# xxayt/MGSV

Hardware: AMD Instinct MI355X
Metric: video-music pairs/s fwd+bwd at B=64 (full training step); sub-objects: retrieval sim-matrix GB/s, eval forward pairs/s (higher is better)
Workload: dtype bf16; 1 GPU; BASELINE.json configs[2]: B=64/GPU, T_v=30, T_a=512, D=512, train mode (dropout on), f32 master weights + Adam, f32 gradient accumulation; global_batch=64, launch=tape

## Files before the change

include/made_hip.h:

```cpp
#ifndef MADE_HIP_H
#define MADE_HIP_H

#include <stdint.h>

#ifdef __cplusplus
extern "C" {
#endif

#define MADE_ABI_VERSION 8

enum MadeDtype { MADE_F32 = 0, MADE_BF16 = 1 };

enum MadeAct {
    MADE_ACT_NONE = 0,
    MADE_ACT_RELU = 1,
    MADE_ACT_GELU = 2,
    MADE_ACT_QUICKGELU = 3,
    MADE_ACT_SIGMOID = 4
};

enum MadeGate {
    MADE_GATE_NONE = 0,
    MADE_GATE_RELU_OUT = 1,
    MADE_GATE_GELU_Z = 2,
// ... 475 lines not shown
                        int64_t B, int64_t T, int64_t F, void* stream);
int made_posbn_relu_bwd(const void* x, int32_t x_dtype, int64_t ldx, const void* y, int32_t y_dtype, int64_t ldy,
                        const void* dy, int32_t dy_dtype, int64_t lddy, const float* weight, const float* save_mean,
                        const float* save_rstd, int32_t batch_stats, void* dx, int32_t dx_dtype, int64_t lddx,
                        float* dweight, float* dbias, int64_t B, int64_t T, int64_t F, void* stream);

int made_set_criterion_bwd(const float* pred_logits, const float* pred_spans, const float* targets,
                           const int64_t* pred_idx, const int64_t* tgt_idx, const int32_t* count,
                           const float* proj_queries, const float* vid_sum, const float* empty_weight,
                           int64_t n_layers, int64_t B, int64_t Q, int64_t G, int64_t Dc, int32_t fg_label,
                           float temperature, const float* weights, const float* upstream,
                           float* d_logits, float* d_spans, int64_t ld_out, int32_t through_sigmoid,
                           float* d_proj_queries, float* d_vid_sum, void* stream);

#define MADE_ADAM_MAX_GROUPS 4
#define MADE_ADAM_NORM_BLOCKS 1024
typedef struct MadeAdamGroup { int64_t begin, end; float lr; float max_norm; } MadeAdamGroup;
int made_adam_step(float* param, const float* grad, float* exp_avg, float* exp_avg_sq, int64_t n,
                   const MadeAdamGroup* groups, int32_t n_groups, float beta1, float beta2, float eps, int64_t step,
                   float grad_scale, float* norm_ws, void* stream);

typedef struct MadeAdamDeviceState { int64_t step; float lr[MADE_ADAM_MAX_GROUPS]; float bc1, bc2_sqrt; } MadeAdamDeviceState;
int made_adam_step_device(float* param, const float* grad, float* exp_avg, float* exp_avg_sq, int64_t n,
                          const MadeAdamGroup* groups, int32_t n_groups, float beta1, float beta2, float eps,
                          MadeAdamDeviceState* state_device, int32_t advance_state, float grad_scale, float* norm_ws, void* stream);

typedef struct MadeRepackDesc {
    const float* src; void* w; void* wt;
    int64_t rows, cols, wt_ld, tile_begin;
    int32_t dtype; int32_t _pad;
} MadeRepackDesc;
int made_repack(const MadeRepackDesc* descs_device, int32_t n_desc, int64_t total_tiles, void* stream);


int made_recall_ranks(const float* sims, int64_t ld, const int32_t* group_id, const int32_t* gt_group, int64_t Nv, int64_t Nm,
                      int64_t n_groups, int32_t* rank_out, int32_t* top1_out, void* stream);

int made_span_iou(const float* pred_logits, const float* pred_spans, const float* gt_moment, const float* m_duration,
                  int64_t N, int64_t Q, int32_t fg_label, float max_m_duration, float* iou_out, float* pred_out, void* stream);

int made_concat_cols(const float* a, int64_t cols_a, const float* c, int64_t cols_c, float* out, int64_t rows, void* stream);


int made_pooled_cosine(const float* anchor, int64_t lda, const void* pooled, int32_t pooled_dtype, float* out, int64_t sa, int64_t sp,
                       int64_t A, int64_t P, int64_t D, void* stream);
int made_scale_exp(const float* x, const float* logit_scale, float* out, int64_t n, void* stream);
int made_span_convert(const float* in, float* out, int64_t N, int32_t mode, void* stream);
int made_span_pairwise(const float* spans1, const float* spans2, float* iou, float* uni, float* giou, float* inter_over_2,
                       int64_t N, int64_t M, void* stream);
int made_span_iou_se(const float* pred_se, const float* gt_moment, const float* m_duration, int64_t N, float max_m_duration,
                     int32_t clamp_to_max, int32_t discounted, float* iou_out, void* stream);


int64_t made_topk_groups_ws_bytes(int64_t Nv, int64_t Nm, int64_t K);
int made_topk_groups(const float* sims, int64_t ld, const int32_t* group_id, int64_t Nv, int64_t Nm, int64_t n_groups,
                     int64_t K, int32_t* idx_out, float* score_out, void* ws, int64_t ws_bytes, void* stream);

int made_gather_pairs(const int32_t* vi, const int32_t* mi, int64_t P, int64_t Nv, int64_t Nm,
                      const void* v_tok, int64_t v_tok_stride, const float* v_mask, int64_t v_mask_stride,
                      const float* v_vec, int64_t v_vec_stride,
                      const void* m_tok, int64_t m_tok_stride, const float* m_mask, int64_t m_mask_stride,
                      const float* m_vec, int64_t m_vec_stride, int64_t Tv, int64_t Ta, int64_t D, int32_t dtype,
                      void* frame_out, int64_t frame_out_stride, void* seg_out, int64_t seg_out_stride,
                      float* fmask_out, float* smask_out, float* video_out, float* music_out, void* stream);


// ... 48 lines not shown
```

mgsv_amd/_lib.py:

```python
from __future__ import annotations

import ctypes as C
import os

_HERE = os.path.dirname(os.path.abspath(__file__))


def variant_env(name: str, default: str = "") -> str:
    if os.environ.get("MADE_DEBUG_VARIANTS", "0") in ("", "0"):
        return default
    return os.environ.get(name, default)


LIB_PATH = os.environ.get("MADE_LIB_PATH") or os.path.join(_HERE, "libmade_hip.so")
ABI_VERSION = 8

F32, BF16 = 0, 1
ACT_NONE, ACT_RELU, ACT_GELU, ACT_QUICKGELU, ACT_SIGMOID = 0, 1, 2, 3, 4
GATE_NONE, GATE_RELU_OUT, GATE_GELU_Z, GATE_QUICKGELU_Z, GATE_SIGMOID_OUT = 0, 1, 2, 3, 4

vp, i64, i32, f32 = C.c_void_p, C.c_int64, C.c_int32, C.c_float

WIDE_PLAN_HEAD, WIDE_PLAN_SAMPLE, WIDE_PLAN_SLOT, WIDE_PLAN_SLOT_BITS = 4, 4, 16, 8

# ... 130 lines not shown

class MadeGemmTNArgs(C.Structure):
    _fields_ = [("A", vp), ("B", vp), ("C", vp), ("ab_dtype", i32), ("c_dtype", i32),
                ("M", i64), ("N", i64), ("K", i64), ("lda", i64), ("ldb", i64), ("ldc", i64),
                ("batch1", i64), ("batch2", i64),
                ("a_zs1", i64), ("a_zs2", i64), ("b_zs1", i64), ("b_zs2", i64), ("c_zs1", i64), ("c_zs2", i64),
                ("row_mask", vp), ("mask_zs1", i64), ("mask_zs2", i64),
                ("alpha", f32), ("accumulate", i32), ("split_m", i64),
                ("colsum", vp), ("colsum_zs1", i64), ("colsum_zs2", i64), ("row_group_valid", vp),
                ("row_index", vp), ("n_rows", vp)]


class MadeGemmTNProblem(C.Structure):
    _fields_ = [("A", vp), ("B", vp), ("C", vp), ("colsum", vp), ("N", i64), ("K", i64), ("lda", i64), ("ldb", i64), ("ldc", i64)]


class MadeGemmTNGroup(C.Structure):
    _fields_ = [("n_problems", i32), ("alpha", f32), ("M", i64), ("split_m", i64), ("row_index", vp), ("n_rows", vp),
                ("p", MadeGemmTNProblem * 8), ("tile_end", i32 * 8), ("tile_size", i32), ("_pad", i32),
                ("workspace", vp), ("workspace_bytes", i64)]


class MadeAdamGroup(C.Structure):
    _fields_ = [("begin", i64), ("end", i64), ("lr", f32), ("max_norm", f32)]


class MadeAdamDeviceState(C.Structure):
    _fields_ = [("step", i64), ("lr", f32 * 4), ("bc1", f32), ("bc2_sqrt", f32)]


class MadeRepackDesc(C.Structure):
    _fields_ = [("src", vp), ("w", vp), ("wt", vp), ("rows", i64), ("cols", i64), ("wt_ld", i64), ("tile_begin", i64),
                ("dtype", i32), ("_pad", i32)]


class MadeFrameDesc(C.Structure):
    _fields_ = [("offset", i64), ("coef", i64), ("H", i32), ("W", i32), ("kh", i32), ("kv", i32)]


class MadeResampleDesc(C.Structure):
    _fields_ = [("offset", i64), ("n", i64), ("taps", i64), ("o", i32), ("m", i32), ("width", i32), ("_pad", i32)]


class MadeAudioSegDesc(C.Structure):
    _fields_ = [("first", i64), ("count", i64)]


SIGNATURES = {
    "made_abi_version": (C.c_int, []),
    "made_set_f32_products": (C.c_int, [C.c_int]),
    "made_get_f32_products": (C.c_int, []),
    "made_last_error": (C.c_char_p, []),
    "made_device_info": (C.c_int, [C.c_char_p, C.c_int, C.POINTER(C.c_int), C.POINTER(C.c_int)]),
    "made_tape_begin": (C.c_int, []),
    "made_tape_end": (C.c_int, [C.POINTER(C.c_uint64)]),
    "made_tape_replay": (C.c_int, [C.c_uint64]),
    "made_tape_free": (C.c_int, [C.c_uint64]),
    "made_tape_interleave": (C.c_int, [C.c_uint64, i32]),
    "made_tape_count": (C.c_int, [C.c_uint64, C.POINTER(i64), C.POINTER(i64), C.POINTER(i64)]),
    "made_tape_replay_range": (C.c_int, [C.c_uint64, i64, i64]),
    "made_tape_op": (C.c_int, [C.c_uint64, i64, C.POINTER(i32), C.POINTER(C.c_uint64), C.POINTER(C.c_uint64), C.POINTER(C.c_uint32)]),
    "made_stream_wait": (C.c_int, [vp, vp]),
    "made_tape_event": (C.c_int, [i32, i32, vp]),
    "made_tape_callback": (C.c_int, [C.CFUNCTYPE(C.c_int, vp), vp]),
    "made_memset_async": (C.c_int, [vp, i32, i64, vp]),
    "made_copy_async": (C.c_int, [vp, vp, i64, vp]),
# ... 12 lines not shown
    "made_layernorm_add": (C.c_int, [vp, i32, i64, vp, vp, vp, i32, i64, vp, i32, i64, vp, i64, i64, i64, f32, vp, vp]),
    "made_cast_mask_rows": (C.c_int, [vp, i64, vp, vp, i32, i64, i64, i64, vp]),
    "made_pack_music_records": (C.c_int, [vp, i32, i64, vp, i64, vp, i64, vp, i32, i64, i64, i64, i64, i64, vp]),
    "made_masked_mean": (C.c_int, [vp, i32, i64, i64, vp, vp, i64, i64, i64, vp]),
    "made_l2norm_rows": (C.c_int, [vp, i32, i64, vp, vp, i32, i64, i64, i64, f32, vp]),
    "made_sine_pe": (C.c_int, [vp, vp, vp, i32, i64, i64, i64, vp]),
    "made_masked_softmax": (C.c_int, [vp, i64, vp, i64, vp, i32, i64, i64, i64, i64, i64, f32, vp]),
    "made_xpool_tail": (C.c_int, [vp, i32, i64, vp, vp, vp, i64, vp, vp, i64, i64, i64, i64, f32, vp]),
    "made_clip_loss": (C.c_int, [vp, i64, i64, vp, f32, i32, vp, vp, vp]),
    "made_hungarian_match": (C.c_int, [vp, vp, vp, i64, i64, i64, i64, i32, f32, f32, f32, vp, i32, vp, vp, vp, vp, vp]),
    "made_attention_bwd": (C.c_int, [C.POINTER(MadeAttnBwdArgs), vp]),
    "made_layernorm_bwd": (C.c_int, [vp, i32, i64, i64, i64, vp, vp, i32, i64, vp, i32, i64, vp, i32, i64, vp, i64,
                                     C.POINTER(MadeDropout), i64, vp, vp, i64, i64, f32, vp, vp]),
    "made_layernorm_bwd2": (C.c_int, [vp, vp, i64, vp, vp, i64, vp, i64, vp, i64, vp, i64, vp, i64, C.POINTER(MadeDropout), i64, i32,
                                      vp, vp, vp, vp, i64, i64, f32, vp]),
    "made_pool_bwd": (C.c_int, [vp, vp, vp, vp, i32, i64, i64, vp, i32, i64, i64, vp, i32, i64, i64, i64, i64, i64, f32, vp]),
    "made_l2norm_bwd": (C.c_int, [vp, i32, i64, vp, i64, i64, vp, i64, i32, vp, i32, i64, i64, i64, f32, vp]),
    "made_clip_loss_bwd": (C.c_int, [vp, i64, i64, vp, f32, vp, vp, vp, vp, i32, vp, vp, vp]),
    "made_xpool_tail_bwd": (C.c_int, [vp, i32, i64, vp, vp, vp, i64, vp, i64, vp, i32, i64, vp, C.POINTER(MadeDropout),
                                      vp, vp, vp, i64, vp, i64, f32, i64, i64, i64, f32, vp]),
    "made_softmax_bwd": (C.c_int, [vp, i64, vp, i64, vp, i64, vp, f32, C.POINTER(MadeDropout), vp, vp, vp, i32, i64, i64,
                                   i64, i64, i64, i64, i64, vp]),
    "made_head_bias": (C.c_int, [vp, i32, i64, vp, vp, i64, i64, i64, vp]),
    "made_head_bias_bwd": (C.c_int, [vp, i32, i64, vp, vp, vp, vp, i64, i64, i64, vp]),
    "made_add3": (C.c_int, [vp, i32, vp, i32, vp, i32, vp, i32, i64, i64, vp]),
    "made_colsum": (C.c_int, [vp, i32, i64, i64, i64, vp, vp]),
    "made_posbn_relu_fwd": (C.c_int, [vp, i32, i64, vp, vp, vp, vp, C.c_float, C.c_float, i32, vp, vp, vp, i32, i64, i64, i64, i64, vp]),
    "made_posbn_relu_bwd": (C.c_int, [vp, i32, i64, vp, i32, i64, vp, i32, i64, vp, vp, vp, i32, vp, i32, i64, vp, vp, i64, i64, i64, vp]),
    "made_set_criterion_bwd": (C.c_int, [vp, vp, vp, vp, vp, vp, vp, vp, vp, i64, i64, i64, i64, i64, i32, f32, vp, vp,
                                         vp, vp, i64, i32, vp, vp, vp]),
    "made_adam_step": (C.c_int, [vp, vp, vp, vp, i64, C.POINTER(MadeAdamGroup), i32, f32, f32, f32, i64, f32, vp, vp]),
    "made_adam_step_device": (C.c_int, [vp, vp, vp, vp, i64, C.POINTER(MadeAdamGroup), i32, f32, f32, f32, vp, i32, f32, vp, vp]),
    "made_repack": (C.c_int, [vp, i32, i64, vp]),
    "made_row_groups": (C.c_int, [vp, i64, vp, vp]),
    "made_row_index": (C.c_int, [vp, i64, vp, vp, vp]),
    "made_linear_variant": (C.c_int, [C.POINTER(MadeLinearArgs)]),
    "made_row_affine": (C.c_int, [vp, i32, i64, vp, vp, i64, i32, vp, i32, i64, i64, i64, vp]),
    "made_gate_rows": (C.c_int, [vp, i32, i64, vp, i32, i64, i32, f32, vp, i64, i64, vp, i32, i64, vp, i64, i64, vp]),
    "made_xpool_fused": (C.c_int, [C.POINTER(MadeXpoolFusedArgs), vp]),
    "made_xpool_attention": (C.c_int, [C.POINTER(MadeXpoolAttnArgs), vp]),
    "made_xpool_sims": (C.c_int, [C.POINTER(MadeXpoolSimsArgs), vp]),
    "made_xpool_sims_ws_bytes": (C.c_int64, [i64, i64, i64]),
    "made_xpool_inbatch": (C.c_int, [C.POINTER(MadeXpoolInbatchArgs), vp]),
    "made_xpool_inbatch_ws_bytes": (C.c_int64, [i64, i64]),
    "made_batch_order": (C.c_int, [vp, i64, i64, vp, vp]),
    "made_recall_ranks": (C.c_int, [vp, i64, vp, vp, i64, i64, i64, vp, vp, vp]),
    "made_span_iou": (C.c_int, [vp, vp, vp, vp, i64, i64, i32, f32, vp, vp, vp]),
    "made_gemm_tn": (C.c_int, [C.POINTER(MadeGemmTNArgs), vp]),
    "made_gemm_tn_grouped": (C.c_int, [C.POINTER(MadeGemmTNGroup), vp]),
    "made_gemm_tn_grouped_workspace": (i64, [C.POINTER(MadeGemmTNGroup)]),
    "made_concat_cols": (C.c_int, [vp, i64, vp, i64, vp, i64, vp]),
    "made_pooled_cosine": (C.c_int, [vp, i64, vp, i32, vp, i64, i64, i64, i64, i64, vp]),
    "made_scale_exp": (C.c_int, [vp, vp, vp, i64, vp]),
    "made_span_convert": (C.c_int, [vp, vp, i64, i32, vp]),
    "made_span_pairwise": (C.c_int, [vp, vp, vp, vp, vp, vp, i64, i64, vp]),
    "made_span_iou_se": (C.c_int, [vp, vp, vp, i64, f32, i32, i32, vp, vp]),
    "made_set_criterion": (C.c_int, [vp, vp, vp, vp, vp, vp, vp, vp, vp, i64, i64, i64, i64, i64, i32, f32, vp, vp, vp, vp]),
    "made_topk_groups_ws_bytes": (C.c_int64, [i64, i64, i64]),
    "made_topk_groups": (C.c_int, [vp, i64, vp, i64, i64, i64, i64, vp, vp, vp, i64, vp]),
    "made_gather_pairs": (C.c_int, [vp, vp, i64, i64, i64, vp, i64, vp, i64, vp, i64, vp, i64, vp, i64, vp, i64, i64, i64, i64, i32,
                                    vp, i64, vp, i64, vp, vp, vp, vp, vp]),
    "made_frames_preprocess": (C.c_int, [vp, i64, vp, i64, vp, i64, vp, i32, i64, vp, vp]),
    "made_audio_resample": (C.c_int, [vp, i64, vp, i64, vp, i64, vp, i64, vp]),
    "made_audio_fbank": (C.c_int, [vp, i64, vp, i64, vp, vp, vp, i32, vp, vp]),
    "made_ast_patches": (C.c_int, [vp, i64, vp, i32, i64, vp]),
}
# ... 39 lines not shown
```

mgsv_amd/csrc/optimizer.hip:

```cpp
#include "common.h"

namespace {

constexpr int OT = 256;

struct AdamArgs {
    float* param; const float* grad; float* m; float* v; int64_t n;
    MadeAdamGroup g[MADE_ADAM_MAX_GROUPS]; int n_groups;
    float beta1, beta2, eps, bc1, bc2_sqrt, grad_scale;
    float* norm_sq;
    const MadeAdamDeviceState* st;
};

__device__ __forceinline__ int group_of(const AdamArgs& a, int64_t i) {
    int gi = -1;
#pragma unroll
    for (int k = 0; k < MADE_ADAM_MAX_GROUPS; ++k)
        if (k < a.n_groups && i >= a.g[k].begin && i < a.g[k].end) gi = k;
    return gi;
}

__global__ __launch_bounds__(OT) void grad_norm_kernel(const AdamArgs a) {
    __shared__ float red[MADE_ADAM_MAX_GROUPS][OT / 64];
    float acc[MADE_ADAM_MAX_GROUPS];
// ... 115 lines not shown
            if (d.w) {
                if (bf && c + 4 <= d.cols && (((r * d.cols + c) & 3) == 0)) {
                    bf16x4 o; o[0] = (bf16_t)v[0]; o[1] = (bf16_t)v[1]; o[2] = (bf16_t)v[2]; o[3] = (bf16_t)v[3];
                    *(bf16x4*)((bf16_t*)d.w + r * d.cols + c) = o;
                } else {
#pragma unroll
                    for (int j = 0; j < 4; ++j) if (c + j < d.cols) store_from_f32(d.w, d.dtype, r * d.cols + c + j, v[j]);
                }
            }
        }
#pragma unroll
        for (int j = 0; j < 4; ++j) tile[rr][4 * tx + j] = v[j];
    }
    __syncthreads();
    if (d.wt) {
#pragma unroll
        for (int k = 0; k < RPT / 16; ++k) {
            const int cc = ty + 16 * k;
            const int64_t c = c0 + cc, r = r0 + 4 * tx;
            if (c < d.cols && r < d.rows) {
                float v[4];
#pragma unroll
                for (int j = 0; j < 4; ++j) v[j] = tile[4 * tx + j][cc];
                if (bf && r + 4 <= d.rows && (((c * d.wt_ld + r) & 3) == 0)) {
                    bf16x4 o; o[0] = (bf16_t)v[0]; o[1] = (bf16_t)v[1]; o[2] = (bf16_t)v[2]; o[3] = (bf16_t)v[3];
                    *(bf16x4*)((bf16_t*)d.wt + c * d.wt_ld + r) = o;
                } else {
#pragma unroll
                    for (int j = 0; j < 4; ++j) if (r + j < d.rows) store_from_f32(d.wt, d.dtype, c * d.wt_ld + r + j, v[j]);
                }
            }
        }
    }
}

}

static int adam_launch(float* param, const float* grad, float* exp_avg, float* exp_avg_sq, int64_t n, const MadeAdamGroup* groups,
                       int32_t n_groups, float beta1, float beta2, float eps, int64_t step, MadeAdamDeviceState* state_device, int advance,
                       float grad_scale, float* norm_ws, void* stream, const char* what) {
    AdamArgs a;
    a.param = param; a.grad = grad; a.m = exp_avg; a.v = exp_avg_sq; a.n = n; a.n_groups = n_groups;
    for (int k = 0; k < MADE_ADAM_MAX_GROUPS; ++k) {
        if (k < n_groups) a.g[k] = groups[k];
        else { a.g[k].begin = a.g[k].end = 0; a.g[k].lr = 0.f; a.g[k].max_norm = 0.f; }
    }
    a.beta1 = beta1; a.beta2 = beta2; a.eps = eps; a.grad_scale = grad_scale;
    a.bc1 = state_device ? 1.f : (float)(1.0 - pow((double)beta1, (double)step));
    a.bc2_sqrt = state_device ? 1.f : (float)sqrt(1.0 - pow((double)beta2, (double)step));
    a.norm_sq = norm_ws;
    a.st = state_device;
    hipStream_t st = (hipStream_t)stream;
    int64_t nb = (n / 4 + OT - 1) / OT;
    if (nb > MADE_ADAM_NORM_BLOCKS) nb = MADE_ADAM_NORM_BLOCKS;
    hipLaunchKernelGGL(grad_norm_kernel, dim3((unsigned)nb), dim3(OT), 0, st, a);
    hipLaunchKernelGGL(norm_finish_kernel, dim3(1), dim3(OT), 0, st, norm_ws, (int)nb, state_device, beta1, beta2, advance);
    hipLaunchKernelGGL(adam_update_kernel, dim3((unsigned)nb), dim3(OT), 0, st, a);
    return made_check_launch(what);
}

extern "C" int made_adam_step(float* param, const float* grad, float* exp_avg, float* exp_avg_sq, int64_t n,
                              const MadeAdamGroup* groups, int32_t n_groups, float beta1, float beta2, float eps, int64_t step,
                              float grad_scale, float* norm_ws, void* stream) {
    MADE_REQUIRE(param && grad && exp_avg && exp_avg_sq && groups && norm_ws, "made_adam_step: null pointer");
    MADE_REQUIRE(n_groups >= 1 && n_groups <= MADE_ADAM_MAX_GROUPS, "made_adam_step: n_groups=%d out of range", n_groups);
    MADE_REQUIRE(n > 0 && n % 4 == 0 && step >= 1, "made_adam_step: n must be a positive multiple of 4 and step >= 1");
    return adam_launch(param, grad, exp_avg, exp_avg_sq, n, groups, n_groups, beta1, beta2, eps, step, nullptr, 0, grad_scale, norm_ws, stream,
                       "made_adam_step");
}

extern "C" int made_adam_step_device(float* param, const float* grad, float* exp_avg, float* exp_avg_sq, int64_t n,
                                     const MadeAdamGroup* groups, int32_t n_groups, float beta1, float beta2, float eps,
                                     MadeAdamDeviceState* state_device, int32_t advance_state, float grad_scale, float* norm_ws, void* stream) {
    MADE_REQUIRE(param && grad && exp_avg && exp_avg_sq && groups && norm_ws && state_device, "made_adam_step_device: null pointer");
    MADE_REQUIRE(n_groups >= 1 && n_groups <= MADE_ADAM_MAX_GROUPS, "made_adam_step_device: n_groups=%d out of range", n_groups);
    MADE_REQUIRE(n > 0 && n % 4 == 0, "made_adam_step_device: n must be a positive multiple of 4");
    return adam_launch(param, grad, exp_avg, exp_avg_sq, n, groups, n_groups, beta1, beta2, eps, 0, state_device, advance_state != 0, grad_scale, norm_ws, stream,
                       "made_adam_step_device");
}

extern "C" int made_repack(const MadeRepackDesc* descs_device, int32_t n_desc, int64_t total_tiles, void* stream) {
    MADE_REQUIRE(descs_device != nullptr && n_desc >= 1 && total_tiles >= 1, "made_repack: bad arguments");
    MADE_UNSUPPORTED(total_tiles < (1LL << 31), "made_repack: too many tiles");
    hipLaunchKernelGGL(repack_kernel, dim3((unsigned)total_tiles), dim3(OT), 0, (hipStream_t)stream, descs_device, (int)n_desc);
    return made_check_launch("made_repack");
}
```

mgsv_amd/trainer.py:

```python
from __future__ import annotations

import math
import os
from typing import Dict, List, Optional, Tuple

import numpy as np
import torch

from . import _lib, dropout as dr, ops, ops_train as tr, tape as _tape
from .config import MadeConfig
from .engine import MadeEngine
from .ops import Seg, round_up

WIDE_SLICES = 8

Tensor = torch.Tensor
XA = "video_guided_to_music_pooling_cross_transformer"


HEAD_PAD = 64


class MadeTrainer(MadeEngine):
    def __init__(self, cfg: MadeConfig, state_dict: Dict[str, object], device="cuda:0", dtype: str = "f32"):
# ... 167 lines not shown
        self.flat_grad = torch.zeros(off, device=dev, dtype=torch.float32)
        self.master: Dict[str, Tensor] = {}
        self.grad: Dict[str, Tensor] = {}
        for k in order:
            n = int(np.prod(shapes[k])) if len(shapes[k]) else 1
            self.master[k] = self.flat_param[offs[k]:offs[k] + n].view(shapes[k])
            self.grad[k] = self.flat_grad[offs[k]:offs[k] + n].view(shapes[k])
            v = sd[k]
            t = v.detach() if isinstance(v, torch.Tensor) else torch.from_numpy(np.asarray(v))
            self.master[k].copy_(t.to(dev, torch.float32))
        self.param_names = order
        self._offs = offs
        self.group_ranges = []
        for gi in range(3):
            ks = [k for k in order if group_of(k) == gi]
            b = offs[ks[0]]
            last = ks[-1]
            e = offs[last] + round_up(int(np.prod(shapes[last])) if len(shapes[last]) else 1, 64)
            self.group_ranges.append((b, e))
        self.exp_avg = torch.zeros_like(self.flat_param)
        self.exp_avg_sq = torch.zeros_like(self.flat_param)
        self.opt_step = 0
        self._norm_ws = torch.zeros(2 * 4 * (1 + 1024), device=dev, dtype=torch.float32)

    def _view(self, store: Dict[str, Tensor], ref) -> Tensor:
        if isinstance(ref, tuple):
            a, b = store[ref[0]], store[ref[1]]
            flat = self.flat_param if store is self.master else self.flat_grad
            o = self._offs[ref[0]]
            rows = a.shape[0] + b.shape[0]
            return flat[o:o + a.numel() + b.numel()].view((rows,) + tuple(a.shape[1:]))
        return store[ref]

    def repack(self, part: Optional[str] = None):
        import ctypes as C
        if getattr(self, "_pack_desc", None) is None:
            P, tc, dev = self.P, self.tc, self.device
            mats, vecs = self._table()
            self.G: Dict[str, Tensor] = {}
            for key, ref in vecs:
                v = self._view(self.master, ref)
                P[key] = v.view(-1) if v.dim() != 1 else v
                g = self._view(self.grad, ref)
                self.G[key] = g.view(-1) if g.dim() != 1 else g
            descs = []
            tiles = 0
            cut = self.group_ranges[0][1]
            part_of = []
            for key, ref in mats:
                m = self._view(self.master, ref)
                self.G[key] = self._view(self.grad, ref)
                rows, cols = m.shape
                w = None
                if tc == torch.float32:
                    P[key] = m
                else:
                    w = torch.empty(rows, cols, device=dev, dtype=tc)
                    P[key] = w
                wt = None
                if key not in ("query_embed", "vit_proj.w", "ast_proj.w"):
                    base = key[:-2] if key.endswith(".w") else key
                    wt = torch.zeros(cols, max(rows, HEAD_PAD), device=dev, dtype=tc)
                    P[base + ".wt"] = wt
                if w is None and wt is None:
                    continue
                d = _lib.MadeRepackDesc()
                d.src, d.w, d.wt = m.data_ptr(), (w.data_ptr() if w is not None else None), (wt.data_ptr() if wt is not None else None)
                d.rows, d.cols, d.wt_ld, d.tile_begin = rows, cols, (wt.shape[1] if wt is not None else 0), tiles
                d.dtype = ops.dt_of(wt if wt is not None else w)
                tiles += ((rows + 63) // 64) * ((cols + 63) // 64)
                descs.append(d)
                part_of.append("rest" if (m.data_ptr() - self.flat_param.data_ptr()) // 4 < cut else "early")

            def pack(ds):
                t0, out = 0, []
                for d in ds:
                    e = _lib.MadeRepackDesc()
                    C.memmove(C.byref(e), C.byref(d), C.sizeof(e))
                    e.tile_begin = t0
                    t0 += ((e.rows + 63) // 64) * ((e.cols + 63) // 64)
                    out.append(e)
                if not out:
                    return None
                arr = (_lib.MadeRepackDesc * len(out))(*out)
                return torch.from_numpy(np.frombuffer(bytes(arr), dtype=np.uint8).copy()).to(dev), len(out), t0
            self._pack_desc = {None: pack(descs), "early": pack([d for d, q in zip(descs, part_of) if q == "early"]),
                               "rest": pack([d for d, q in zip(descs, part_of) if q == "rest"])}
        pk = self._pack_desc[part]
        if pk is not None:
            _lib.check(_lib.lib().made_repack(pk[0].data_ptr(), pk[1], pk[2], torch.cuda.current_stream().cuda_stream), "made_repack")
        if self.cfg.agg_module == "mlp" and part != "early":
            P = self.P
            for key, mod, _ in self._mlp_towers():
                for bn in ("1", "4"):
                    sc, sh = P[f"{key}.{bn}.scale"], P[f"{key}.{bn}.shift"]
                    torch.add(self.buffers[f"{mod}.net.{bn}.running_var"], 1e-5, out=sc)
                    sc.rsqrt_().mul_(P[f"{key}.{bn}.g"])
                    torch.mul(self.buffers[f"{mod}.net.{bn}.running_mean"], sc, out=sh)
                    sh.neg_().add_(P[f"{key}.{bn}.beta"])

    def optimizer_step(self, lr_temporal: float, lr_matching: float, lr_detection: float, max_grad_norm: float = 1.0,
                       betas=(0.9, 0.999), eps: float = 1e-8, grad_scale: float = 1.0, device_state: Optional[Tensor] = None,
                       part: Optional[str] = None) -> None:
        import ctypes as C
        assert part in (None, "early", "rest")
        if part != "rest":
            self.opt_step += 1
            self.generation += 1
        groups = (_lib.MadeAdamGroup * 3)()
        for i, lr in enumerate((lr_temporal, lr_matching, lr_detection)):
            groups[i].begin, groups[i].end = self.group_ranges[i]
            if (part == "early" and i == 0) or (part == "rest" and i != 0):
                groups[i].end = groups[i].begin
            groups[i].lr, groups[i].max_norm = float(lr), float(max_grad_norm)
        ws = self._norm_ws[:self._norm_ws.numel() // 2] if part != "early" else self._norm_ws[self._norm_ws.numel() // 2:]
        if device_state is not None:
            _lib.check(_lib.lib().made_adam_step_device(self.flat_param.data_ptr(), self.flat_grad.data_ptr(), self.exp_avg.data_ptr(),
                                                        self.exp_avg_sq.data_ptr(), self.flat_param.numel(), groups, 3, float(betas[0]),
                                                        float(betas[1]), float(eps), device_state.data_ptr(), 0 if part == "rest" else 1,
                                                        float(grad_scale), ws.data_ptr(), torch.cuda.current_stream().cuda_stream),
                       "made_adam_step_device")
            self.repack(part)
            return
        _lib.check(_lib.lib().made_adam_step(self.flat_param.data_ptr(), self.flat_grad.data_ptr(), self.exp_avg.data_ptr(),
                                             self.exp_avg_sq.data_ptr(), self.flat_param.numel(), groups, 3, float(betas[0]), float(betas[1]),
                                             float(eps), self.opt_step, float(grad_scale), ws.data_ptr(),
                                             torch.cuda.current_stream().cuda_stream), "made_adam_step")
        self.repack(part)

    def train_step(self, frame_feats, segment_feats, frame_masks, segment_masks, spans_target, seed: int, lrs=(1e-4, 1e-4, 1e-4),
                   max_grad_norm: float = 1.0, w_ret: Optional[Tensor] = None, w_loc: Optional[Tensor] = None, dist=None,
                   music_ids=None, v_duration: Optional[Tensor] = None) -> Dict[str, Tensor]:
        self._zero_grad_in_forward = True
        try:
            out = self.forward_train(frame_feats, segment_feats, frame_masks, segment_masks, spans_target, seed=seed, music_ids=music_ids,
                                     v_duration=v_duration)
        finally:
            self._zero_grad_in_forward = False
        scale = 1.0
        if dist is not None and dist.get_world_size() > 1:
            cut = self.group_ranges[0][1]
            works = []
            self.backward(w_ret, w_loc, grad_sync=lambda: works.append(dist.all_reduce(self.flat_grad[cut:], async_op=True)))
            works.append(dist.all_reduce(self.flat_grad[:cut], async_op=True))
            for w in works:
                w.wait()
            scale = 1.0 / dist.get_world_size()
        elif self._early_opt_ok():
# ... 760 lines not shown
                                 ld_out=HEAD_PAD, through_sigmoid=True)
            hs2 = ws["hs"].view(nd * B * Q, D)
            dhs = tw["dhs"]
            dlog, dsp = tw["dlog"], tw["dsp"]
            if self.tc != torch.float32:
                tr.add3(tw["dlogsp_c"], tw["dlogsp"])
                dlog, dsp = tw["dlog_c"], tw["dsp_c"]
            heads_dw: list = []
            heads_dw.append(lambda: tr.gemm_tn(dlog[:, :2], hs2, G["class_embed.w"], accumulate=True, colsum=G["class_embed.b"]))
            ops.linear(dlog, P["class_embed.wt"], None, out=dhs)
            n_span = 1 if c.predict_center == 1 else 2
            heads_dw.append(lambda: tr.gemm_tn(dsp[:, :n_span], tw["h2"], G["span_embed.2.w"], accumulate=True, colsum=G["span_embed.2.b"]))
            dz2 = ops.linear(dsp, P["span_embed.2.wt"], None, out=tw["hg1"], gate=_lib.GATE_RELU_OUT, G=tw["h2"])
            dz1 = self._lin_bwd(dz2, tw["h1"], "span_embed.1", dx_out=tw["hg2"], gate=_lib.GATE_RELU_OUT, G=tw["h1"], later=heads_dw)
            self._lin_bwd(dz1, hs2, "span_embed.0", dx_out=dhs, R=dhs, later=heads_dw)
            if c.contrastive_align_loss:
                Dc = pq.shape[-1]
                dn = tw["dpq"]
                if c.audio_short_cut:
                    if c.aux_loss and nd > 1:
                        n_aux = (nd - 1) * B * Q
                        ds2 = tw["dpq_s2"][:n_aux]
                        tr.l2norm_bwd(tw["pq_s2"][:n_aux], dn[:n_aux], dx=ds2)
                        dmusic.add_(ds2.view(nd - 1, B, Q, D).sum((0, 2)))
                        dn[:n_aux].copy_(ds2)
                    tr.l2norm_bwd(tw["pq_s1"], dn, dx=tw["dpq_s"])
                    dmusic.add_(tw["dpq_s"].view(nd, B, Q, D).sum((0, 2)))
                    dn = tw["dpq_s"]
                tr.l2norm_bwd(ws["pq_raw"], dn, dx_alt=tw["dpq_raw"])
                self._lin_bwd(tw["dpq_raw"], hs2, "proj_q", dx_out=dhs, R=dhs, later=heads_dw)
                tr.l2norm_bwd(ws["pv_raw"], tw["dvid_sum"], dx_alt=tw["dpv_raw"], dy_rows_per=Tv)
                heads_dw.append(lambda: tr.gemm_tn(tw["dpv_raw"][:Tv], frame[0], G["proj_v.w"], accumulate=True, colsum=G["proj_v.b"], batch=(B, 1),
                                                   a_zs=(Tv * Dc, 0), b_zs=(frame.stride(0), 0), colsum_zs=(0, 0)))
                ops.linear(tw["dpv_raw"], P["proj_v.wt"], None, out=tw["dframe_x"])

            qp = P["query_embed"]
            mem3, mempos3 = tw["mem"].view(B, L, D), tw["mempos"].view(B, L, D)
            Lp = tw["PdS"].shape[-1]
            GQ, PdS = tw["GQ"], tw["PdS"]
            ca_scale = 1.0 / math.sqrt(hd)
            st = tw["dstack"]
            dtgt = None
            stage = self._dec_stage_chain()
            pre = bool(c.detr_pre_norm)
            S_all = tw["dS_S"]
            if not stage:
                ops.linear(GQ[0, 1].reshape(nd * HQ, D), mempos3[0], None, M=nd * HQ, N=L, K=D, batch=B, a_z_stride=GQ.stride(0), w_z_stride=L * D,
                           segs=[Seg(out=S_all, ldo=Lp, rows_per_batch=HQ, out_batch_stride=B * HQ * Lp, out_z_stride=HQ * Lp)])
            n_split_b = int(_lib.variant_env("MADE_WIDE_NSPLIT", "0")) or max(1, min(8, 256 // max(B, 1)))
            wplan = self._wide_plan if HQ <= 8 and _lib.variant_env("MADE_WIDE_PLANNED", "1") != "0" else None
            if wplan is not None:
                n_split_b = WIDE_SLICES
            if stage:
                gN = tw["dgN"]
                tr.layernorm_bwd(tw["dstack"]["tgt"][1:].reshape(nd * B * Q, D), P["dec.norm.g"], dhs, gN, dgamma=G["dec.norm.g"], dbeta=G["dec.norm.b"])
            for l in range(nd - 1, -1, -1):
                p, d = f"detr_transformer.decoder.layers.{l}", f"d.{l}"
                g1, g2, g4 = tw["dg1"], tw["dg2"], tw["dg4"]
                if stage and _lib.variant_env("MADE_CHAIN_BUFS", "1") != "0":
                    ch = tw["dchain"][l]
                    g1a, g1b, g2a, g2b, g2c, dt_out = ch[0], ch[1], ch[2], ch[3], ch[4], ch[5]
                else:
                    g1a = g1b = g1
                    g2a = g2b = g2c = g2
                    dt_out = tw["dtgt"]
                Win, Wt = P[p + ".ca.in.w"], P[p + ".ca.in.wt"]
                g_ffn, g_z, g_ca, g_attc, g_q, g_qc, g_sa, gqkv = (st[k][l] for k in ("g_ffn", "g_z", "g_ca", "g_attc", "g_q", "g_qc", "g_sa", "g_qkv"))
# ... 798 lines not shown
```

Before: 14160 pairs/s.

## Fuse Adam update with weight repack into a single tiled optimizer kernel

```diff
diff --git a/include/made_hip.h b/include/made_hip.h
--- a/include/made_hip.h
+++ b/include/made_hip.h
@@ -531,6 +531,13 @@
 } MadeRepackDesc;
 int made_repack(const MadeRepackDesc* descs_device, int32_t n_desc, int64_t total_tiles, void* stream);
 
+typedef struct MadeOptUnit { int64_t begin; int32_t n; int32_t desc; int32_t group; int32_t _pad; } MadeOptUnit;
+int made_adam_repack_step_device(float* param, const float* grad, float* exp_avg, float* exp_avg_sq, int64_t n,
+                                 const MadeAdamGroup* groups, int32_t n_groups, float beta1, float beta2, float eps,
+                                 MadeAdamDeviceState* state_device, float grad_scale, float* norm_ws,
+                                 const MadeRepackDesc* descs_device, int32_t n_desc, const MadeOptUnit* units_device, int32_t n_units,
+                                 void* stream);
+
 
 int made_recall_ranks(const float* sims, int64_t ld, const int32_t* group_id, const int32_t* gt_group, int64_t Nv, int64_t Nm,
                       int64_t n_groups, int32_t* rank_out, int32_t* top1_out, void* stream);
diff --git a/mgsv_amd/_lib.py b/mgsv_amd/_lib.py
--- a/mgsv_amd/_lib.py
+++ b/mgsv_amd/_lib.py
@@ -186,6 +186,10 @@
 class MadeRepackDesc(C.Structure):
     _fields_ = [("src", vp), ("w", vp), ("wt", vp), ("rows", i64), ("cols", i64), ("wt_ld", i64), ("tile_begin", i64),
                 ("dtype", i32), ("_pad", i32)]
+
+
+class MadeOptUnit(C.Structure):
+    _fields_ = [("begin", i64), ("n", i32), ("desc", i32), ("group", i32), ("_pad", i32)]
 
 
 class MadeFrameDesc(C.Structure):
@@ -264,6 +268,8 @@
     "made_adam_step": (C.c_int, [vp, vp, vp, vp, i64, C.POINTER(MadeAdamGroup), i32, f32, f32, f32, i64, f32, vp, vp]),
     "made_adam_step_device": (C.c_int, [vp, vp, vp, vp, i64, C.POINTER(MadeAdamGroup), i32, f32, f32, f32, vp, i32, f32, vp, vp]),
     "made_repack": (C.c_int, [vp, i32, i64, vp]),
+    "made_adam_repack_step_device": (C.c_int, [vp, vp, vp, vp, i64, C.POINTER(MadeAdamGroup), i32, f32, f32, f32, vp, f32, vp,
+                                               vp, i32, vp, i32, vp]),
     "made_row_groups": (C.c_int, [vp, i64, vp, vp]),
     "made_row_index": (C.c_int, [vp, i64, vp, vp, vp]),
     "made_linear_variant": (C.c_int, [C.POINTER(MadeLinearArgs)]),
diff --git a/mgsv_amd/csrc/optimizer.hip b/mgsv_amd/csrc/optimizer.hip
--- a/mgsv_amd/csrc/optimizer.hip
+++ b/mgsv_amd/csrc/optimizer.hip
@@ -171,6 +171,252 @@
             }
         }
     }
+}
+
+
+struct FusedArgs {
+    AdamArgs a;
+    const MadeRepackDesc* descs;
+    const MadeOptUnit* units;
+    int nblocks;
+    int fold;
+};
+
+constexpr int NU = 4;
+
+__global__ __launch_bounds__(OT) void grad_norm_ahead_kernel(const AdamArgs a, MadeAdamDeviceState* st, float beta1, float beta2, int advance) {
+#pragma clang fp contract(off)
+    __shared__ float red[MADE_ADAM_MAX_GROUPS][OT / 64];
+    if (advance && blockIdx.x == 0 && threadIdx.x == 0) {
+        const int64_t step = ++st->step;
+        st->bc1 = (float)(1.0 - pow((double)beta1, (double)step));
+        st->bc2_sqrt = (float)sqrt(1.0 - pow((double)beta2, (double)step));
+    }
+    float acc[MADE_ADAM_MAX_GROUPS];
+#pragma unroll
+    for (int k = 0; k < MADE_ADAM_MAX_GROUPS; ++k) acc[k] = 0.f;
+    const int64_t stride = (int64_t)gridDim.x * OT * 4;
+    for (int64_t i0 = ((int64_t)blockIdx.x * OT + threadIdx.x) * 4; i0 < a.n; i0 += stride * NU) {
+        f32x4 g4[NU];
+        int gi[NU];
+#pragma unroll
+        for (int u = 0; u < NU; ++u) {
+            const int64_t i = i0 + stride * u;
+            gi[u] = i < a.n ? group_of(a, i) : -1;
+            g4[u] = f32x4{0.f, 0.f, 0.f, 0.f};
+            if (gi[u] >= 0) g4[u] = *(const f32x4*)(a.grad + i);
+        }
+#pragma unroll
+        for (int u = 0; u < NU; ++u) {
+            if (gi[u] < 0) continue;
+#pragma unroll
+            for (int j = 0; j < 4; ++j) {
+                const float g = g4[u][j] * a.grad_scale;
+                const float sq = g * g;
+#pragma unroll
+                for (int k = 0; k < MADE_ADAM_MAX_GROUPS; ++k) acc[k] += (gi[u] == k) ? sq : 0.f;
+            }
+        }
+    }
+    const int lane = threadIdx.x & 63, wave = threadIdx.x >> 6;
+#pragma unroll
+    for (int k = 0; k < MADE_ADAM_MAX_GROUPS; ++k) {
+        const float s = wave_sum(acc[k]);
+        if (lane == 0) red[k][wave] = s;
+    }
+    __syncthreads();
+    if (threadIdx.x < MADE_ADAM_MAX_GROUPS) {
+        float s = 0.f;
+        for (int w = 0; w < OT / 64; ++w) s += red[threadIdx.x][w];
+        a.norm_sq[MADE_ADAM_MAX_GROUPS + (int64_t)blockIdx.x * MADE_ADAM_MAX_GROUPS + threadIdx.x] = s;
+    }
+}
+
+__device__ __forceinline__ void adam_elem(float graw, float& p, float& m, float& v, float grad_scale, float cf, float beta1, float beta2,
+                                          float omb1, float omb2, float lr_bc1, float bc2_sqrt, float eps) {
+#pragma clang fp contract(off)
+    const float g = graw * grad_scale * cf;
+    const float t = g * (g * omb2);
+    v = __builtin_fmaf(beta2, v, t);
+    m = __builtin_fmaf(beta1, m, omb1 * g);
+    const float denom = sqrtf(v) / bc2_sqrt + eps;
+    p = __builtin_fmaf(-lr_bc1, m / denom, p);
+}
+
+__device__ __forceinline__ f32x4 ld4(const float* p, bool vec, int nvalid) {
+    if (vec) return *(const f32x4*)p;
+    f32x4 q = {0.f, 0.f, 0.f, 0.f};
+#pragma unroll
+    for (int j = 0; j < 4; ++j) if (j < nvalid) q[j] = p[j];
+    return q;
+}
+__device__ __forceinline__ void st4(float* p, const f32x4 q, bool vec, int nvalid) {
+    if (vec) { *(f32x4*)p = q; return; }
+#pragma unroll
+    for (int j = 0; j < 4; ++j) if (j < nvalid) p[j] = q[j];
+}
+
+__device__ __forceinline__ void fold_norms(const FusedArgs& f, float (*red)[MADE_ADAM_MAX_GROUPS], float* s_cf, float* s_lr) {
+#pragma clang fp contract(off)
+    const AdamArgs& a = f.a;
+    float s[MADE_ADAM_MAX_GROUPS];
+#pragma unroll
+    for (int k = 0; k < MADE_ADAM_MAX_GROUPS; ++k) s[k] = 0.f;
+    static_assert(MADE_ADAM_MAX_GROUPS == 4, "the partials of one workgroup are read as one 16-byte vector");
+    for (int b = threadIdx.x; b < (f.fold ? f.nblocks : 0); b += OT) {
+        const f32x4 q = *(const f32x4*)(a.norm_sq + MADE_ADAM_MAX_GROUPS + (int64_t)b * MADE_ADAM_MAX_GROUPS);
+#pragma unroll
+        for (int k = 0; k < MADE_ADAM_MAX_GROUPS; ++k) s[k] += q[k];
+    }
+#pragma unroll
+    for (int k = 0; k < MADE_ADAM_MAX_GROUPS; ++k) red[threadIdx.x][k] = s[k];
+    __syncthreads();
+    for (int o = f.fold ? OT / 2 : 0; o > 0; o >>= 1) {
+        if (threadIdx.x < o) {
+#pragma unroll
+            for (int k = 0; k < MADE_ADAM_MAX_GROUPS; ++k) red[threadIdx.x][k] += red[threadIdx.x + o][k];
+        }
+        __syncthreads();
+    }
+    if (threadIdx.x < MADE_ADAM_MAX_GROUPS) {
+        const int k = threadIdx.x;
+        const float nsq = f.fold ? red[0][k] : a.norm_sq[k];
+        if (f.fold && blockIdx.x == 0) a.norm_sq[k] = nsq;
+        float cf = 1.f;
+        if (k < a.n_groups && a.g[k].max_norm > 0.f) {
+            const float c = a.g[k].max_norm / (sqrtf(nsq) + 1e-6f);
+            cf = c < 1.f ? c : 1.f;
+        }
+        s_cf[k] = cf;
+        s_lr[k] = a.st->lr[k] / a.st->bc1;
+    }
+    __syncthreads();
+}
+
+template <bool FULL>
+__device__ __forceinline__ void tile_unit(const FusedArgs& f, const MadeOptUnit& u, const MadeRepackDesc& d, float (*tile)[RPT + 1],
+                                          float (*red)[MADE_ADAM_MAX_GROUPS], float* s_cf, float* s_lr) {
+    const AdamArgs& a = f.a;
+    const bool upd = u.group >= 0;
+    const float omb1 = 1.f - a.beta1, omb2 = 1.f - a.beta2;
+    const int64_t tc_n = (d.cols + RPT - 1) / RPT;
+    const int64_t r0 = (u.begin / tc_n) * RPT, c0 = (u.begin % tc_n) * RPT;
+    const int tx = threadIdx.x & 15, ty = threadIdx.x >> 4;
+    const bool bf = d.dtype == MADE_BF16;
+    const int64_t base = d.src - a.param;
+    f32x4 g4[RPT / 16], p4[RPT / 16], m4[RPT / 16], v4[RPT / 16];
+#pragma unroll
+    for (int k = 0; k < RPT / 16; ++k) {
+        const int64_t r = r0 + ty + 16 * k, c = c0 + 4 * tx;
+        p4[k] = f32x4{0.f, 0.f, 0.f, 0.f};
+        if (FULL || (r < d.rows && c < d.cols)) {
+            const int64_t i = base + r * d.cols + c;
+            const bool vec = FULL || (c + 4 <= d.cols && ((i & 3) == 0));
+            const int nv = FULL ? 4 : (int)(d.cols - c < 4 ? d.cols - c : 4);
+            p4[k] = ld4(a.param + i, vec, nv);
+            if (upd) { g4[k] = ld4(a.grad + i, vec, nv); m4[k] = ld4(a.m + i, vec, nv); v4[k] = ld4(a.v + i, vec, nv); }
+        }
+    }
+    if (upd || blockIdx.x == 0) fold_norms(f, red, s_cf, s_lr);
+    float cf = 1.f, lr_bc1 = 0.f, bc2_sqrt = 1.f;
+    if (upd) { cf = s_cf[u.group]; lr_bc1 = s_lr[u.group]; bc2_sqrt = a.st->bc2_sqrt; }
+#pragma unroll
+    for (int k = 0; k < RPT / 16; ++k) {
+        const int rr = ty + 16 * k;
+        const int64_t r = r0 + rr, c = c0 + 4 * tx;
+        float v[4] = {0.f, 0.f, 0.f, 0.f};
+        if (FULL || (r < d.rows && c < d.cols)) {
+            const int64_t i = base + r * d.cols + c;
+            const bool vec = FULL || (c + 4 <= d.cols && ((i & 3) == 0));
+            const int nv = FULL ? 4 : (int)(d.cols - c < 4 ? d.cols - c : 4);
+            if (upd) {
+#pragma unroll
+                for (int j = 0; j < 4; ++j) {
+                    if (j >= nv) continue;
+                    float p = p4[k][j], m = m4[k][j], w = v4[k][j];
+                    adam_elem(g4[k][j], p, m, w, a.grad_scale, cf, a.beta1, a.beta2, omb1, omb2, lr_bc1, bc2_sqrt, a.eps);
+                    p4[k][j] = p; m4[k][j] = m; v4[k][j] = w;
+                }
+                st4(a.m + i, m4[k], vec, nv); st4(a.v + i, v4[k], vec, nv); st4(a.param + i, p4[k], vec, nv);
+            }
+            v[0] = p4[k][0]; v[1] = p4[k][1]; v[2] = p4[k][2]; v[3] = p4[k][3];
+            if (d.w) {
+                if (bf && c + 4 <= d.cols && (((r * d.cols + c) & 3) == 0)) {
+                    bf16x4 o; o[0] = (bf16_t)v[0]; o[1] = (bf16_t)v[1]; o[2] = (bf16_t)v[2]; o[3] = (bf16_t)v[3];
+                    *(bf16x4*)((bf16_t*)d.w + r * d.cols + c) = o;
+                } else {
+#pragma unroll
+                    for (int j = 0; j < 4; ++j) if (c + j < d.cols) store_from_f32(d.w, d.dtype, r * d.cols + c + j, v[j]);
+                }
+            }
+        }
+#pragma unroll
+        for (int j = 0; j < 4; ++j) tile[rr][4 * tx + j] = v[j];
+    }
+    __syncthreads();
+    if (d.wt) {
+#pragma unroll
+        for (int k = 0; k < RPT / 16; ++k) {
+            const int cc = ty + 16 * k;
+            const int64_t c = c0 + cc, r = r0 + 4 * tx;
+            if (c < d.cols && r < d.rows) {
+                float v[4];
+#pragma unroll
+                for (int j = 0; j < 4; ++j) v[j] = tile[4 * tx + j][cc];
+                if (bf && r + 4 <= d.rows && (((c * d.wt_ld + r) & 3) == 0)) {
+                    bf16x4 o; o[0] = (bf16_t)v[0]; o[1] = (bf16_t)v[1]; o[2] = (bf16_t)v[2]; o[3] = (bf16_t)v[3];
+                    *(bf16x4*)((bf16_t*)d.wt + c * d.wt_ld + r) = o;
+                } else {
+#pragma unroll
+                    for (int j = 0; j < 4; ++j) if (r + j < d.rows) store_from_f32(d.wt, d.dtype, c * d.wt_ld + r + j, v[j]);
+                }
+            }
+        }
+    }
+}
+
+__global__ __launch_bounds__(OT) void adam_repack_kernel(const FusedArgs f) {
+    __shared__ float tile[RPT][RPT + 1];
+    __shared__ float red[OT][MADE_ADAM_MAX_GROUPS];
+    __shared__ float s_cf[MADE_ADAM_MAX_GROUPS], s_lr[MADE_ADAM_MAX_GROUPS];
+    const AdamArgs& a = f.a;
+    const MadeOptUnit u = f.units[blockIdx.x];
+    if (u.desc < 0) {
+        const float omb1 = 1.f - a.beta1, omb2 = 1.f - a.beta2;
+        f32x4 g4[4], p4[4], m4[4], v4[4];
+        bool on[4];
+#pragma unroll
+        for (int k = 0; k < 4; ++k) {
+            const int e = (threadIdx.x + OT * k) * 4;
+            on[k] = u.group >= 0 && e < u.n;
+            if (on[k]) {
+                const int64_t i = u.begin + e;
+                g4[k] = *(const f32x4*)(a.grad + i); p4[k] = *(const f32x4*)(a.param + i);
+                m4[k] = *(const f32x4*)(a.m + i); v4[k] = *(const f32x4*)(a.v + i);
+            }
+        }
+        fold_norms(f, red, s_cf, s_lr);
+        if (u.group < 0) return;
+        const float cf = s_cf[u.group], lr_bc1 = s_lr[u.group], bc2_sqrt = a.st->bc2_sqrt;
+#pragma unroll
+        for (int k = 0; k < 4; ++k) {
+            if (!on[k]) continue;
+            const int64_t i = u.begin + (threadIdx.x + OT * k) * 4;
+#pragma unroll
+            for (int j = 0; j < 4; ++j) {
+                float p = p4[k][j], m = m4[k][j], v = v4[k][j];
+                adam_elem(g4[k][j], p, m, v, a.grad_scale, cf, a.beta1, a.beta2, omb1, omb2, lr_bc1, bc2_sqrt, a.eps);
+                p4[k][j] = p; m4[k][j] = m; v4[k][j] = v;
+            }
+            *(f32x4*)(a.m + i) = m4[k]; *(f32x4*)(a.v + i) = v4[k]; *(f32x4*)(a.param + i) = p4[k];
+        }
+        return;
+    }
+    const MadeRepackDesc d = f.descs[u.desc];
+    const int64_t tc_n = (d.cols + RPT - 1) / RPT;
+    const int64_t r0 = (u.begin / tc_n) * RPT, c0 = (u.begin % tc_n) * RPT;
+    if (r0 + RPT <= d.rows && c0 + RPT <= d.cols && (d.cols & 3) == 0 && (((d.src - a.param) & 3) == 0)) tile_unit<true>(f, u, d, tile, red, s_cf, s_lr);
+    else tile_unit<false>(f, u, d, tile, red, s_cf, s_lr);
 }
 
 }
@@ -224,3 +470,40 @@
     hipLaunchKernelGGL(repack_kernel, dim3((unsigned)total_tiles), dim3(OT), 0, (hipStream_t)stream, descs_device, (int)n_desc);
     return made_check_launch("made_repack");
 }
+
+extern "C" int made_adam_repack_step_device(float* param, const float* grad, float* exp_avg, float* exp_avg_sq, int64_t n,
+                                            const MadeAdamGroup* groups, int32_t n_groups, float beta1, float beta2, float eps,
+                                            MadeAdamDeviceState* state_device, float grad_scale, float* norm_ws,
+                                            const MadeRepackDesc* descs_device, int32_t n_desc, const MadeOptUnit* units_device,
+                                            int32_t n_units, void* stream) {
+    MADE_REQUIRE(param && grad && exp_avg && exp_avg_sq && groups && norm_ws && state_device && descs_device && units_device,
+                 "made_adam_repack_step_device: null pointer");
+    MADE_REQUIRE(n_groups >= 1 && n_groups <= MADE_ADAM_MAX_GROUPS, "made_adam_repack_step_device: n_groups=%d out of range", n_groups);
+    MADE_REQUIRE(n > 0 && n % 4 == 0 && n_desc >= 1 && n_units >= 1, "made_adam_repack_step_device: n must be a positive multiple of 4, n_desc and n_units >= 1");
+    MADE_REQUIRE(((((uintptr_t)param) | ((uintptr_t)grad) | ((uintptr_t)exp_avg) | ((uintptr_t)exp_avg_sq) | ((uintptr_t)norm_ws)) & 15) == 0,
+                 "made_adam_repack_step_device: the flat buffers and norm_ws must be 16-byte aligned");
+    FusedArgs f;
+    AdamArgs& a = f.a;
+    a.param = param; a.grad = grad; a.m = exp_avg; a.v = exp_avg_sq; a.n = n; a.n_groups = n_groups;
+    for (int k = 0; k < MADE_ADAM_MAX_GROUPS; ++k) {
+        if (k < n_groups) a.g[k] = groups[k];
+        else { a.g[k].begin = a.g[k].end = 0; a.g[k].lr = 0.f; a.g[k].max_norm = 0.f; }
+        MADE_REQUIRE(a.g[k].begin % 4 == 0 && a.g[k].end % 4 == 0 && a.g[k].begin >= 0 && a.g[k].end <= n && a.g[k].begin <= a.g[k].end,
+                     "made_adam_repack_step_device: group %d: bounds must be multiples of 4 inside [0, n]", k);
+    }
+    a.beta1 = beta1; a.beta2 = beta2; a.eps = eps; a.grad_scale = grad_scale;
+    a.bc1 = 1.f; a.bc2_sqrt = 1.f;
+    a.norm_sq = norm_ws;
+    a.st = state_device;
+    f.descs = descs_device; f.units = units_device;
+    hipStream_t st = (hipStream_t)stream;
+    int64_t nb = (n / 4 + OT - 1) / OT;
+    if (nb > MADE_ADAM_NORM_BLOCKS) nb = MADE_ADAM_NORM_BLOCKS;
+    f.nblocks = (int)nb;
+    const char* fold_env = made_variant_env("MADE_OPT_FOLD");
+    f.fold = !(fold_env && fold_env[0] == '0');
+    hipLaunchKernelGGL(grad_norm_ahead_kernel, dim3((unsigned)nb), dim3(OT), 0, st, a, state_device, beta1, beta2, 1);
+    if (!f.fold) hipLaunchKernelGGL(norm_finish_kernel, dim3(1), dim3(OT), 0, st, norm_ws, (int)nb, state_device, beta1, beta2, 0);
+    hipLaunchKernelGGL(adam_repack_kernel, dim3((unsigned)n_units), dim3(OT), 0, st, f);
+    return made_check_launch("made_adam_repack_step_device");
+}
diff --git a/mgsv_amd/trainer.py b/mgsv_amd/trainer.py
--- a/mgsv_amd/trainer.py
+++ b/mgsv_amd/trainer.py
@@ -223,7 +223,7 @@
             return flat[o:o + a.numel() + b.numel()].view((rows,) + tuple(a.shape[1:]))
         return store[ref]
 
-    def repack(self, part: Optional[str] = None):
+    def repack(self, part: Optional[str] = None, launch: bool = True):
         import ctypes as C
         if getattr(self, "_pack_desc", None) is None:
             P, tc, dev = self.P, self.tc, self.device
@@ -277,9 +277,12 @@
                 return torch.from_numpy(np.frombuffer(bytes(arr), dtype=np.uint8).copy()).to(dev), len(out), t0
             self._pack_desc = {None: pack(descs), "early": pack([d for d, q in zip(descs, part_of) if q == "early"]),
                                "rest": pack([d for d, q in zip(descs, part_of) if q == "rest"])}
-        pk = self._pack_desc[part]
-        if pk is not None:
-            _lib.check(_lib.lib().made_repack(pk[0].data_ptr(), pk[1], pk[2], torch.cuda.current_stream().cuda_stream), "made_repack")
+            self._pack_host = descs
+            self.optimizer_units()
+        if launch:
+            pk = self._pack_desc[part]
+            if pk is not None:
+                _lib.check(_lib.lib().made_repack(pk[0].data_ptr(), pk[1], pk[2], torch.cuda.current_stream().cuda_stream), "made_repack")
         if self.cfg.agg_module == "mlp" and part != "early":
             P = self.P
             for key, mod, _ in self._mlp_towers():
@@ -289,6 +292,58 @@
                     sc.rsqrt_().mul_(P[f"{key}.{bn}.g"])
                     torch.mul(self.buffers[f"{mod}.net.{bn}.running_mean"], sc, out=sh)
                     sh.neg_().add_(P[f"{key}.{bn}.beta"])
+
+    def optimizer_units(self):
+        if getattr(self, "_opt_units", False) is not False:
+            return self._opt_units
+        self._opt_units = None
+        descs = self._pack_host
+        if not descs or self._pack_desc[None] is None:
+            return None
+        p0, n_flat = self.flat_param.data_ptr(), self.flat_param.numel()
+        units, covered = [], []
+        for di, d in enumerate(descs):
+            off, n = (int(d.src) - p0) // 4, int(d.rows) * int(d.cols)
+            assert (int(d.src) - p0) % 4 == 0 and 0 <= off and off + n <= n_flat
+            gi = [k for k, (b, e) in enumerate(self.group_ranges) if b <= off and off + n <= e]
+            if not gi and not all(off + n <= b or e <= off for b, e in self.group_ranges):
+                return None
+            if gi and (off % 4 or n % 4):
+                return None
+            for t in range(((int(d.rows) + 63) // 64) * ((int(d.cols) + 63) // 64)):
+                units.append((t, 0, di, gi[0] if gi else -1))
+            if gi:
+                covered.append((off, off + n))
+        covered.sort()
+        if any(a[1] > b[0] for a, b in zip(covered, covered[1:])):
+            return None
+        for k, (b, e) in enumerate(self.group_ranges):
+            assert b % 4 == 0 and e % 4 == 0
+            at = b
+            for cb, ce in [c for c in covered if b <= c[0] < e] + [(e, e)]:
+                assert cb >= at, "matrices overlap"
+                while at < cb:
+                    n = min(4096, cb - at)
+                    units.append((at, n, -1, k))
+                    at += n
+                at = max(at, ce)
+        host = np.asarray(units, dtype=np.int64).reshape(-1, 4)
+        cnt = np.zeros(n_flat + 1, dtype=np.int32)
+        for (cb, ce) in covered:
+            cnt[cb] += 1; cnt[ce] -= 1
+        sp = host[host[:, 2] < 0]
+        np.add.at(cnt, sp[:, 0], 1); np.add.at(cnt, sp[:, 0] + sp[:, 1], -1)
+        cnt = np.cumsum(cnt[:-1])
+        want = np.zeros(n_flat, dtype=np.int32)
+        for b, e in self.group_ranges:
+            want[b:e] += 1
+        assert np.array_equal(cnt, want), "optimizer units do not partition the groups' ranges"
+        arr = np.zeros(len(host), dtype=np.dtype([("begin", "<i8"), ("n", "<i4"), ("desc", "<i4"), ("group", "<i4"), ("_pad", "<i4")]))
+        assert arr.dtype.itemsize == __import__("ctypes").sizeof(_lib.MadeOptUnit)
+        arr["begin"], arr["n"], arr["desc"], arr["group"] = host[:, 0], host[:, 1], host[:, 2], host[:, 3]
+        dev = torch.from_numpy(np.frombuffer(arr.tobytes(), dtype=np.uint8).copy()).to(self.device)
+        self._opt_units = (dev, len(host), host)
+        return self._opt_units
 
     def optimizer_step(self, lr_temporal: float, lr_matching: float, lr_detection: float, max_grad_norm: float = 1.0,
                        betas=(0.9, 0.999), eps: float = 1e-8, grad_scale: float = 1.0, device_state: Optional[Tensor] = None,
@@ -305,6 +360,15 @@
                 groups[i].end = groups[i].begin
             groups[i].lr, groups[i].max_norm = float(lr), float(max_grad_norm)
         ws = self._norm_ws[:self._norm_ws.numel() // 2] if part != "early" else self._norm_ws[self._norm_ws.numel() // 2:]
+        if device_state is not None and part is None and _lib.variant_env("MADE_OPT_FUSED", "1") != "0" and self.optimizer_units() is not None:
+            un, pk = self.optimizer_units(), self._pack_desc[None]
+            _lib.check(_lib.lib().made_adam_repack_step_device(self.flat_param.data_ptr(), self.flat_grad.data_ptr(), self.exp_avg.data_ptr(),
+                                                               self.exp_avg_sq.data_ptr(), self.flat_param.numel(), groups, 3, float(betas[0]),
+                                                               float(betas[1]), float(eps), device_state.data_ptr(), float(grad_scale),
+                                                               ws.data_ptr(), pk[0].data_ptr(), pk[1], un[0].data_ptr(), un[1],
+                                                               torch.cuda.current_stream().cuda_stream), "made_adam_repack_step_device")
+            self.repack(launch=False)
+            return
         if device_state is not None:
             _lib.check(_lib.lib().made_adam_step_device(self.flat_param.data_ptr(), self.flat_grad.data_ptr(), self.exp_avg.data_ptr(),
                                                         self.exp_avg_sq.data_ptr(), self.flat_param.numel(), groups, 3, float(betas[0]),
@@ -1131,7 +1195,11 @@
                 tr.l2norm_bwd(ws["pv_raw"], tw["dvid_sum"], dx_alt=tw["dpv_raw"], dy_rows_per=Tv)
                 heads_dw.append(lambda: tr.gemm_tn(tw["dpv_raw"][:Tv], frame[0], G["proj_v.w"], accumulate=True, colsum=G["proj_v.b"], batch=(B, 1),
                                                    a_zs=(Tv * Dc, 0), b_zs=(frame.stride(0), 0), colsum_zs=(0, 0)))
-                ops.linear(tw["dpv_raw"], P["proj_v.wt"], None, out=tw["dframe_x"])
+                dframe = lambda: ops.linear(tw["dpv_raw"], P["proj_v.wt"], None, out=tw["dframe_x"])
+                if _lib.variant_env("MADE_DFRAME_LATE", "1") != "0":
+                    heads_dw.append(dframe)
+                else:
+                    dframe()
 
             qp = P["query_embed"]
             mem3, mempos3 = tw["mem"].view(B, L, D), tw["mempos"].view(B, L, D)
```

Result: faster. 14320 pairs/s (median of 6 runs) (+1.1%).
